# HaoruXue/spline-trajectory-optimization

Measured on AMD Instinct MI355X. Metric: min-curvature QP solves/sec (N=2000 waypoints), higher is better.
Workload: dtype f64

## Files before the change

spline_trajectory_optimization_amd/csrc/rl_device.hpp:

```cpp
#pragma once
#include <hip/hip_runtime.h>
#include "rl_sep.hpp"

namespace rl {

constexpr int kWave = 64;
constexpr int kMaxK = 5;

struct TrackDev {
  int k, n, nt, N;
  const double* t;
  const double* c0;
  const int* ell;
  const double* D;
  const int* sup;
  const double* base;
  const double* Ds;
  const double* base_s;
};

template <int K>
__device__ __forceinline__ void deboor(const double* __restrict__ t, double x, int l, int m,
                                       double (&h)[K + 1]) {
  double hh[K + 1];
// ... 195 lines not shown
      v = ring[j1];
      const double bx = v.x - px, by = v.y - py;
      const double eb = edge_side<ST>(bx, by, dx, dy);
      edge_hit<ST>(ax, ay, ea, bx, by, eb, dx, dy, j, h);
      ax = bx; ay = by; ea = eb;
      j = j1;
    }
  }
}

constexpr int kChunk = 8;
constexpr int kWinChunks = 3;
constexpr int kNear = 1;
constexpr int kWinEdges = kWinChunks * kChunk;
constexpr int kRingPad = kWinEdges + 1;
constexpr int kWinBatch = 8;

template <int BATCH = kWinBatch, bool ST = false, typename RingPtr>
__device__ __forceinline__ void scan_window(RingPtr ring, int nr, int lo, int lo_edge, double px, double py,
                                            double dx, double dy, Hit& h, const double* cmax_p,
                                            unsigned long long* counts = nullptr) {
  unsigned cand;
  {
    unsigned signs;
    double emin;
    bool sure;
    {
      const double c0 = fma(px, dy, -(py * dx));
      double2 v = ring[lo];
      const double e0 = fma(v.x, dy, fma(-v.y, dx, -c0));
      signs = (unsigned)__double2hiint(e0) >> 31;
      emin = fabs(e0);
#pragma unroll
      for (int q0 = 0; q0 < kWinEdges; q0 += BATCH) {
        double2 w[BATCH];
#pragma unroll
        for (int u = 0; u < BATCH; ++u) w[u] = ring[lo + q0 + u + 1];
#pragma unroll
        for (int u = 0; u < BATCH; ++u) {
          const double eb = fma(w[u].x, dy, fma(-w[u].y, dx, -c0));
          signs = __builtin_amdgcn_alignbit(signs, (unsigned)__double2hiint(eb), 31);
// ... 18 lines not shown
        double2 w[BATCH];
#pragma unroll
        for (int u = 0; u < BATCH; ++u) w[u] = ring[lo + q0 + u + 1];
#pragma unroll
        for (int u = 0; u < BATCH; ++u) {
          const double eb = edge_side<ST>(w[u].x - px, w[u].y - py, dx, dy);
          signs = __builtin_amdgcn_alignbit(signs, (unsigned)__double2hiint(eb), 31);
          emin = fmin(emin, fabs(eb));
        }
        if constexpr (BATCH != kWinBatch) __builtin_amdgcn_sched_barrier(0);
      }
      sure = emin != 0.0;
    }
    cand = __builtin_bitreverse32((signs ^ (signs >> 1)) & 0xFFFFFFu) >> 8;
    if (!sure) cand = 0xFFFFFFu;
    const bool sides_known = !__any(!sure);
    static_assert(kWinEdges == 24 && kWinEdges % BATCH == 0, "window scan is unrolled in whole batches; the candidate word holds 24 edges");
    while (__any(cand != 0u)) {
#ifdef RL_STAMPS
      if (counts) counts[2] += 1;
#endif
      if (cand != 0u) {
        const int q = __ffs((int)cand) - 1;
        cand &= cand - 1u;
        const int j = lo + q, je = lo_edge + q;
        const double2 va = ring[j], vb = ring[j + 1];
        const double ax = va.x - px, ay = va.y - py, bx = vb.x - px, by = vb.y - py;
        if (sides_known) edge_cross<ST>(ax, ay, bx, by, dx, dy, je >= nr ? je - nr : je, h);
        else edge_hit<ST>(ax, ay, edge_side<ST>(ax, ay, dx, dy), bx, by, edge_side<ST>(bx, by, dx, dy), dx, dy,
                          je >= nr ? je - nr : je, h);
      }
    }
  }
}

constexpr int kStage = 96;
constexpr int kStageBatch = 8;
static_assert(kStage >= kWinEdges + 1 + 64 && kStage <= 104, "a stretch holds the windows of 64 consecutive chunk starts; two DMA instructions fill it");
constexpr int kStageSlots = kStage + kStage / kChunk;
__device__ __forceinline__ int stage_slot(int v) { return v + (v >> 3); }

__device__ __forceinline__ void stage_issue(const double2* ring, int nr, int base, double2* stg, int lane) {
  static_assert(kStageSlots > kWave && kStageSlots <= 2 * kWave, "two instructions cover the stretch");
#pragma unroll
  for (int t0 = 0; t0 <= kStageSlots - kWave; t0 += kStageSlots - kWave) {
    const int t = t0 + lane;
    const int v = t - t / 9;
    int idx = base + (v < kStage ? v : kStage - 1);
    if (idx >= nr) idx -= nr;
    __builtin_amdgcn_global_load_lds((const __attribute__((address_space(1))) void*)(ring + idx),
                                     (__attribute__((address_space(3))) void*)(stg + t0), 16, 0, 0);
  }
}
struct StagedWindow {
  const double2* p;
  __device__ __forceinline__ double2 operator[](int k) const { return p[k + (k >> 3)]; }
};
__device__ __forceinline__ void stage_wait() {
  asm volatile("s_waitcnt vmcnt(0)" ::: "memory");
  __builtin_amdgcn_fence(__ATOMIC_ACQUIRE, "wavefront");
}
__device__ __forceinline__ int window_start(int hint, int nchunk) {
  int cs = hint / kChunk - 1;
  if (cs < 0) cs += nchunk;
  return cs * kChunk;
}

__device__ __forceinline__ int stage_prefetch(const double2* ring, int nr, int nchunk, bool active, int hint, double2* stg, int lane) {
  const unsigned long long m = __ballot(active && hint >= 0 && hint < nr);
  const int first = m ? __ffsll((long long)m) - 1 : 0;
  const int lo = __builtin_amdgcn_readlane(window_start(hint, nchunk), first);
  const int base = m ? lo : 0;
  asm volatile("s_waitcnt lgkmcnt(0)" ::: "memory");
  stage_issue(ring, nr, base, stg, lane);
  return base;
}

template <bool ST = false, typename RingPtr>
__device__ __forceinline__ Hit search_ring_brute(RingPtr ring, int nr, double px, double py,
                                                 double dx, double dy) {
  Hit h{INFINITY, 0.0, kNoEdge};
  scan_edges<ST>(ring, nr, 0, nr, px, py, dx, dy, h);
  return h;
}


template <bool ST = false, typename RingPtr, typename CirclePtr>
__device__ __forceinline__ Hit search_ring_culled(RingPtr ring, int nr, CirclePtr circ, int nchunk,
                                                  double px, double py, double dx, double dy,
// ... 46 lines not shown
    v = Op::f(v, __hiloint2double(hi_, lo_));                                                                   \
  }
  RL_BFLY(0x041F) RL_BFLY(0x081F) RL_BFLY(0x101F) RL_BFLY(0x201F) RL_BFLY(0x401F)
#undef RL_BFLY
  const int other = (((int)threadIdx.x ^ 32) & 63) << 2;
  const int lo_ = __builtin_amdgcn_ds_bpermute(other, __double2loint(v));
  const int hi_ = __builtin_amdgcn_ds_bpermute(other, __double2hiint(v));
  return Op::f(v, __hiloint2double(hi_, lo_));
}
__device__ __forceinline__ double wave_max_bfly(double v) { return wave_reduce_bfly<OpMax>(v); }
__device__ __forceinline__ double wave_min_bfly(double v) { return wave_reduce_bfly<OpMin>(v); }
__device__ __forceinline__ double wave_sum(double v) { return wave_reduce<OpSum>(v); }
__device__ __forceinline__ double wave_max(double v) { return wave_reduce<OpMax>(v); }
__device__ __forceinline__ double wave_min(double v) { return wave_reduce<OpMin>(v); }

template <bool STAGED = false, bool ST = false, typename RingPtr, typename CirclePtr>
__device__ __forceinline__ Hit search_ring_windowed(RingPtr ring, int nr, CirclePtr circ,
                                                    CirclePtr sep, int nchunk, bool active, int hint,
                                                    double px, double py, double dx, double dy,
                                                    double dlen, const double* cmax, bool skip_guard = false,
                                                    unsigned long long* stamps = nullptr,
                                                    double2* stg = nullptr, int staged_base = -1) {
  const int lane = threadIdx.x & (kWave - 1);
  Hit h{INFINITY, 0.0, kNoEdge};
  const bool windowed = active && hint >= 0 && hint < nr;
  const int lo = window_start(hint, nchunk);
#ifdef RL_STAMPS
  unsigned long long w0 = 0, w1 = 0;
  asm volatile("s_memtime %0\n\ts_waitcnt lgkmcnt(0)" : "=s"(w0) :: "memory");
#endif
  if constexpr (!STAGED) {
    if (windowed) scan_window<kWinBatch, ST>(ring, nr, lo, lo, px, py, dx, dy, h, cmax);
  } else {
    bool todo = windowed;
    int base = staged_base;
    if (base >= 0) stage_wait();
    for (;;) {
      if (base >= 0) {
        int off = lo - base;
        if (off < 0) off += nr;
        if (todo && (off & (kChunk - 1)) == 0 && off + kWinEdges + 1 <= kStage) {
          scan_window<kStageBatch, ST>(StagedWindow{stg + stage_slot(off)}, nr, 0, lo, px, py, dx, dy, h, cmax, stamps);
          todo = false;
        }
      }
      const unsigned long long left = __ballot(todo);
      if (left == 0ull) break;
      base = __builtin_amdgcn_readlane(lo, __ffsll((long long)left) - 1);
      asm volatile("s_waitcnt lgkmcnt(0)" ::: "memory");
      stage_issue(reinterpret_cast<const double2*>(ring), nr, base, stg, lane);
      stage_wait();
    }
  }
#ifdef RL_STAMPS
  asm volatile("s_waitcnt vmcnt(0)\n\ts_memtime %0\n\ts_waitcnt lgkmcnt(0)" : "=s"(w1) :: "memory");
  if (stamps) stamps[0] += w1 - w0;
#endif
  if (skip_guard) return h;
  const bool found = h.best <= 1.0;
  const double di = active ? ((found ? h.best * dlen : dlen) * (1.0 + 1e-9) + 1e-9) : 0.0;
  auto chunk_in_window = [&](int c) {
    const int e0 = c * kChunk;
    const int cnt = min(kChunk, nr - e0);
    int off = e0 - lo;
    if (off < 0) off += nr;
// ... 67 lines not shown
```

spline_trajectory_optimization_amd/csrc/rl_host.hpp:

```cpp
#pragma once

#include "../../include/rl_mincurv.h"

#include <hip/hip_runtime.h>

#include <mutex>
#include <string>
#include <utility>
#include <vector>

namespace {

thread_local std::string g_err;

int fail(int code, const std::string& msg) {
  g_err = msg;
  return code;
}

#define RL_HIP(expr)                                                                      \
  do {                                                                                    \
    hipError_t _e = (expr);                                                               \
    if (_e != hipSuccess) {                                                               \
      return fail(RL_ERR_HIP, std::string(#expr) + ": " + hipGetErrorString(_e));         \
// ... 23 lines not shown
};

}

struct rl_ctx {
  int device = 0;
  hipStream_t stream = nullptr;
  hipEvent_t ev0 = nullptr, ev1 = nullptr;
  int max_lds = 65536;
  int num_cu = 0;
  bool force_global_v1 = false;
  int arith = RL_ARITH_REFERENCE;
  bool arith_explicit = false;
  int np_raise_at_start = 0;
  int qss_kernel = -1, qss_df_waves = 4, qss_df_bail_at = 0, qss_df_redo = 1;
  int tables_search = RL_SEARCH_WINDOWED, tables_rings_global = 0;
  int frenet_search = 1;
  void* arena = nullptr;
  size_t arena_cap = 0;
  hipEvent_t arena_ev = nullptr;
  hipStream_t arena_stream = nullptr;
  bool arena_busy = false;
  static constexpr int kMaxGroups = 8;
  hipStream_t aux_stream[kMaxGroups - 1] = {};
  hipEvent_t ev_fork = nullptr, ev_join[kMaxGroups - 1] = {};
  hipStream_t poll_stream = nullptr;
  hipEvent_t ev_chunk[kMaxGroups] = {}, ev_poll[2] = {nullptr, nullptr};
  double* poll_host = nullptr;
  size_t poll_cap = 0;
  bool mt_hes_sweep = false;
// ... 207 lines not shown
```

spline_trajectory_optimization_amd/csrc/rl_mincurv.hip:

```cpp
#include "rl_host.hpp"

#include <algorithm>
#include <cmath>
#include <cstdio>
#include <cstdlib>
#include <cstring>
#include <type_traits>

#include "rl_kernels.hpp"
#include "rl_sweep.hpp"
#include "rl_qss_df.hpp"
#include "rl_global.hpp"
#include "rl_global2.hpp"
#include "rl_global_xy.hpp"
#include "rl_dtrack.hpp"
#include "rl_mintime.hpp"
#include "rl_bicycle.hpp"
#include "rl_region.hpp"
#include "rl_tables.hpp"
#include "rl_pose_tables.hpp"
#include "rl_spline_fit.hpp"
#include "rl_frenet.hpp"

namespace {
// ... 78 lines not shown
  int want = B >= 2 * ctx->num_cu ? 0 : 1;
  if (force && (force[0] == '0' || force[0] == '1')) want = force[0] == '1' ? 0 : 1;
  if (const char* r = getenv("RL_FORCE_RESIDENCY")) if (r[0] >= '0' && r[0] <= '2') want = r[0] - '0';
  if (strict && want == 2) want = 0;
  rl::SweepLds in = rl::sweep_lds_layout(n, N, nL, nR, Residency::Lds, joint, strict);
  if (want == 1 && in.total * sizeof(double) > (size_t)ctx->max_lds) want = 0;
  if (want == 2) {
    rl::SweepLds mid = rl::sweep_lds_layout(n, N, nL, nR, Residency::CrossingsLds, joint);
    if (mid.total * sizeof(double) > (size_t)ctx->max_lds) want = 0;
  }
  p.residency = want == 1 ? Residency::Lds : want == 2 ? Residency::CrossingsLds : Residency::Global;
  rl::SweepLds L = rl::sweep_lds_layout(n, N, nL, nR, p.residency, joint, strict);
  p.lds_bytes = L.total * sizeof(double);
  const size_t per_sample_arrays = rl::sweep_keeps_table_xy(joint, strict) ? 3 : 2;
  p.gscratch_doubles = (p.residency != Residency::Global ? 0 : per_sample_arrays * ((N + 1) & ~1) * (strict ? 2 : 1)) +
                       (p.residency == Residency::Lds ? 0 : (size_t)2 * (nL + rl::kRingPad) + (size_t)2 * (nR + rl::kRingPad));
  return p;
}

constexpr bool kRecordSteps = true;
template <int K, rl::Driver DRIVER, rl::Arith ARITH, bool DUMP = false>
int launch_sweep_in(const rl_ctx* ctx, const SweepPlan& p, const rl::SweepArgs& a) {
  using rl::Residency; using rl::SweepConfig;
  const dim3 grid(a.B), block(rl::kSweepThreads);
  return p.residency == Residency::Lds
             ? launch(ctx, rl::k_sweep<SweepConfig<K, Residency::Lds, DRIVER, ARITH, DUMP>>, grid, block, p.lds_bytes, a)
             : launch(ctx, rl::k_sweep<SweepConfig<K, Residency::Global, DRIVER, ARITH, DUMP>>, grid, block, p.lds_bytes, a);
}

int launch_sweep(const rl_ctx* ctx, int k, const SweepPlan& p, const rl::SweepArgs& a, bool joint = false, bool strict = false,
                 bool lite = false) {
// ... 208 lines not shown
    return fail(RL_ERR_ARG, "arith must be RL_ARITH_DEFAULT, RL_ARITH_FAST, RL_ARITH_REFERENCE or RL_ARITH_BRANCH");
  ctx->arith = arith;
  ctx->arith_explicit = true;
  return RL_OK;
}

int rl_ctx_get_arith(const rl_ctx* ctx) { return ctx ? (ctx->arith_explicit ? ctx->arith : RL_ARITH_DEFAULT) : RL_ERR_ARG; }

int rl_ctx_set_option(rl_ctx* ctx, const char* name, int value) {
  if (!ctx || !name) return fail(RL_ERR_ARG, "null argument");
  const std::string k(name);
  if (k == "qss_kernel") { if (value < -1 || value > 1) return fail(RL_ERR_ARG, "qss_kernel: -1 (auto), 0 (list order), 1 (dataflow)"); ctx->qss_kernel = value; }
  else if (k == "qss_df_waves") { if (value != 1 && value != 2 && value != 4) return fail(RL_ERR_ARG, "qss_df_waves: 1, 2 or 4"); ctx->qss_df_waves = value; }
  else if (k == "qss_df_bail_at") { if (value < 0) return fail(RL_ERR_ARG, "qss_df_bail_at >= 0"); ctx->qss_df_bail_at = value; }
  else if (k == "qss_df_redo") { if (value != 0 && value != 1) return fail(RL_ERR_ARG, "qss_df_redo: 0 or 1"); ctx->qss_df_redo = value; }
  else if (k == "tables_search") { if (value < RL_SEARCH_BRUTE || value > RL_SEARCH_WINDOWED) return fail(RL_ERR_ARG, "tables_search: RL_SEARCH_BRUTE, _CULLED or _WINDOWED"); ctx->tables_search = value; }
  else if (k == "tables_rings") { if (value != 0 && value != 1) return fail(RL_ERR_ARG, "tables_rings: 0 (LDS where they fit) or 1 (arena)"); ctx->tables_rings_global = value; }
  else if (k == "frenet_search") { if (value != 0 && value != 1) return fail(RL_ERR_ARG, "frenet_search: 0 (table bound for every point) or 1 (from the previous point's piece)"); ctx->frenet_search = value; }
  else return fail(RL_ERR_ARG, "unknown option '" + k + "'");
  return RL_OK;
}

int rl_ctx_set_numpy_raise(rl_ctx* ctx, int on) {
  if (!ctx) return fail(RL_ERR_ARG, "ctx is null");
  ctx->np_raise_at_start = on ? 1 : 0;
  return RL_OK;
}

int rl_debug_cr_heading(rl_ctx* ctx, const double* dx, const double* dy, int n, double* out) {
  if (!ctx || !dx || !dy || !out || n <= 0) return fail(RL_ERR_ARG, "bad argument");
// ... 221 lines not shown
    RL_HIP(hipSetDevice(ctx->device));
    if (int rc = ensure_strict_tables(ctx, trk)) return rc;
  }
  rl::SweepArgs a;
  std::memset(&a, 0, sizeof(a));
  a.tr = trk->dev();
  a.B = B;
  a.form = form;
  a.in = in_dev;
  Bounds bd;
  if (int rc = resolve_bounds(trk, form, in_dev, bd)) return rc;
  a.ringL = bd.ringL; a.ringR = bd.ringR; a.nL = bd.nL; a.nR = bd.nR;
  a.max_iter = max_iter;
  for (int j = 0; j < max_iter && !i_start_rows; ++j) a.i_start[j] = i_start[j];
  a.ctrl0 = ctrl0; a.i_start_rows = i_start_rows;
  a.search = search;
  a.max_dist = 100.0;
#ifdef RL_ABLATION
  if (const char* dbg = getenv("RL_DEBUG_FLAGS")) a.debug = atoi(dbg);
#endif
#ifdef RL_STAMPS
  const bool dbg_ok = true;
#else
  const bool dbg_ok = !strict;
#endif
  if (g_dbg_instances > 0 && (joint || k == 5) && dbg_ok && !from) {
    const int ninst = std::min(g_dbg_instances, B);
    size_t need = joint ? (size_t)max_iter * (size_t)(i_max - i_min) * (48 + 9 * rl::kJointRowsPerThread * 256 + 2 * n)
                        : (size_t)ninst * max_iter * 2 * (size_t)(i_max - i_min) * (rl::kSweepDumpHead + 2 * n);
#ifdef RL_STAMPS
    need = std::max(need, (size_t)B * 4 * 17);
#endif
    a.dbg_instances = ninst;
    if (g_dbg_len < need) {
      if (g_dbg_buf) (void)hipFree(g_dbg_buf);
      RL_HIP(hipMalloc(reinterpret_cast<void**>(&g_dbg_buf), need * sizeof(double)));
      g_dbg_len = need;
    }
    RL_HIP(hipMemsetAsync(g_dbg_buf, 0, need * sizeof(double), ctx->stream));
    a.dbg = g_dbg_buf;
  }
  a.out_ctrl = out_ctrl; a.out_xy = out_xy; a.out_points = out_points;
  a.n_success = n_success; a.status = status;
  RL_HIP(hipSetDevice(ctx->device));
  SweepPlan p = plan_sweep(ctx, n, N, a.nL, a.nR, B, joint, strict);
  if (p.lds_bytes > (size_t)ctx->max_lds) return fail(RL_ERR_UNSUPPORTED, "problem does not fit LDS");
// ... 1203 lines not shown
```

spline_trajectory_optimization_amd/csrc/rl_sweep.hpp:

```cpp
#pragma once
#include "rl_kernels.hpp"

namespace rl {

constexpr int kJointRowsPerThread = 3;

struct SweepArgs {
  TrackDev tr;
  int B;
  int form;
  const double* in;
  const double2* ringL;
  const double2* ringR;
  int nL, nR;
  int max_iter;
  int i_start[32];
  int search;
  double max_dist;
  double* out_ctrl;
  double* out_xy;
  double* out_points;
  int* n_success;
  int* status;
  double* gscratch;
  size_t gscratch_stride;
  double* dbg;
  int dbg_instances;
  int debug;
  int np_raise_at_start;
  double* aux;
  size_t aux_stride;
  int* n_raised;
  int* raise_flag;
  const double* ctrl0;
  const int* i_start_rows;
};

#ifdef RL_STAMPS
#define RL_STAMP(var) do { __builtin_amdgcn_sched_barrier(0); asm volatile("s_memtime %0\n\ts_waitcnt lgkmcnt(0)" : "=s"(var) :: "memory"); __builtin_amdgcn_sched_barrier(0); } while (0)
#define RL_STAMP_ADD(slot, t1, t0) st_acc[slot] += (t1) - (t0)
#define RL_STRICT_COUNTS st_cnt
#define RL_FSTAMP(slot) do { RL_STAMP(sf1); st_fine[slot] += sf1 - sf0; sf0 = sf1; } while (0)
#else
#define RL_STAMP(var) do { } while (0)
#define RL_STAMP_ADD(slot, t1, t0) do { } while (0)
#define RL_STRICT_COUNTS nullptr
#define RL_FSTAMP(slot) do { } while (0)
#endif

#ifdef RL_ABLATION
#define RL_ABLATE(a, bit) (((a).debug & (bit)) != 0)
#else
#define RL_ABLATE(a, bit) false
#endif

enum class Residency { Lds, Global, CrossingsLds };

struct SweepLds {
  int cpad, nLp, nRp, ncL, ncR;
  size_t off_cx, off_cy, off_red, off_sL, off_sR, off_rL, off_rR, off_cL, off_cR, off_pL, off_pR, off_hint, off_joint, off_stage,
         off_c12, off_terms, off_pxy, total;
};
__host__ __device__ constexpr bool sweep_keeps_table_xy(bool joint, bool strict) { return strict && !joint; }
constexpr int kSweepWaves = 4;
constexpr int kSweepThreads = kWave * kSweepWaves;
constexpr int kTermChunk = 256;
constexpr int kTermStride = kTermChunk + 2;
constexpr int kC12Doubles = 4 * (2 * kMaxK) + 8;
constexpr int kRedCoordMax = 194;
constexpr int kRedRadiusMax = 192;

__host__ __device__ inline SweepLds sweep_lds_layout(int n, int N, int nL, int nR, Residency residency,
                                                     bool joint = false, bool strict = false) {
  const bool rings_in_lds = residency == Residency::Lds, sigma_in_lds = residency != Residency::Global;
  SweepLds L;
  L.cpad = (n + 1) & ~1;
  L.nLp = nL; L.nRp = nR;
  L.ncL = (nL + kChunk - 1) / kChunk;
  L.ncR = (nR + kChunk - 1) / kChunk;
// ... 55 lines not shown
};
template <Residency RESIDENCY, Arith ARITH = Arith::Fast>
struct SweepConfigWindowFrom : SweepConfig<5, RESIDENCY, Driver::Window, ARITH, false> {
  static_assert(RESIDENCY != Residency::CrossingsLds, "the sliding-window driver: all-LDS or all-global residency");
  static constexpr bool from = true;
};

template <class Cfg>
__global__ __launch_bounds__(kSweepThreads, Cfg::workgroups_per_cu) void k_sweep(SweepArgs a) {
  constexpr int K = Cfg::K, BLOCK = kSweepThreads, NW = kSweepWaves;
  constexpr bool RINGS_LDS = Cfg::residency == Residency::Lds, SIGMA_LDS = Cfg::residency != Residency::Global;
  constexpr bool JOINT = Cfg::driver == Driver::Window, DUMP = Cfg::DUMP;
  constexpr bool STRICT = Cfg::arith != Arith::Fast, RAISE = Cfg::arith == Arith::ReferenceRaise, LITE = Cfg::arith == Arith::Branch;
  constexpr bool STAGED = !RINGS_LDS;
  constexpr bool FROM = Cfg::from;
  if constexpr (RAISE) { if (!a.raise_flag || a.raise_flag[blockIdx.x] == 0) return; }
#ifdef RL_STAMPS
  unsigned long long st_entry = 0;
  RL_STAMP(st_entry);
#endif
  extern __shared__ __attribute__((aligned(16))) unsigned char smem_raw[];
  double* smem = reinterpret_cast<double*>(smem_raw);
  const TrackDev& tr = a.tr;
  const int n = tr.n, N = tr.N;
  const int b = blockIdx.x;
  const int tid = threadIdx.x;
  const int lane = tid % kWave, wave = tid / kWave;
  const SweepLds L = sweep_lds_layout(n, N, a.nL, a.nR, Cfg::residency, JOINT, STRICT);
  double2* stgL = reinterpret_cast<double2*>(smem + L.off_stage) + (STAGED ? wave * 2 * kStageSlots : 0);
  double2* stgR = stgL + kStageSlots;
// ... 106 lines not shown
          m = v <= 0x1p+1000 ? fmax(m, v) : INFINITY;
          rm = o[2] <= 0x1p+1000 ? fmax(rm, o[2]) : INFINITY;
        }
        m = wave_max_bfly(m);
        rm = wave_max_bfly(rm);
        if (lane == 0) { red[kRedCoordMax] = m; red[kRedRadiusMax] = rm; }
      }
      __syncthreads();
      const double rmax = red[kRedRadiusMax];
      for (int c = tid; c < L.ncL + L.ncR; c += BLOCK) {
        const bool left = c < L.ncL;
        const int cc = left ? c : c - L.ncL;
        (left ? sepL : sepR)[cc] = chunk_separation(left ? circL : circR, left ? L.ncL : L.ncR, cc, kNear, rmax);
      }
      __syncthreads();
    }
  }

  double* jq = smem + L.off_joint;
  unsigned char* outside = reinterpret_cast<unsigned char*>(jq + 128);
  int* n_outside = reinterpret_cast<int*>(jq + 127);
  auto note_outside = [&](int i, double px, double py, double ndx, double ndy, double sl, double sr) {
    const double Lx = px + sl * ndx, Ly = py + sl * ndy;
    const double Rx = px + sr * (-ndx), Ry = py + sr * (-ndy);
    const bool out = fmin(Lx, Rx) > px || fmax(Lx, Rx) < px || fmin(Ly, Ry) > py || fmax(Ly, Ry) < py;
    const int was = outside[i];
    if ((int)out != was) { outside[i] = out ? 1 : 0; atomicAdd(n_outside, out ? 1 : -1); }
  };
  auto note_outside_pts = [&](int i, double px, double py, double2 Lp, double2 Rp) {
    const bool out = fmin(Lp.x, Rp.x) > px || fmax(Lp.x, Rp.x) < px || fmin(Lp.y, Rp.y) > py || fmax(Lp.y, Rp.y) < py;
    const int was = outside[i];
    if ((int)out != was) { outside[i] = out ? 1 : 0; atomicAdd(n_outside, out ? 1 : -1); }
  };
  if (JOINT) {
    for (int i = tid; i < N; i += BLOCK) outside[i] = 0;
    if (tid == 0) *n_outside = 0;
    __syncthreads();
  }

#ifdef RL_STAMPS
  unsigned long long st_cnt[4] = {0, 0, 0, 0};
  unsigned long long st_fine[8] = {0, 0, 0, 0, 0, 0, 0, 0}, sf0 = 0, sf1 = 0;
#endif
  unsigned char* degen = (RAISE && a.aux) ? reinterpret_cast<unsigned char*>(a.aux + (size_t)b * a.aux_stride + 2 * L.cpad) : nullptr;
  int* n_degen = reinterpret_cast<int*>(red + 190);
  bool flag_mode = false;
  bool saw_degenerate = false;
  auto refresh = [&](int i0, int i1, int j0, int j1, int mode, int l_first = -1, bool from_base = false) {
    const int m0 = i1 - i0, m1 = j1 - j0, m = m0 + m1;
    const double* cmax = red + kRedCoordMax;
    if constexpr (STRICT) {
      int delta = 0;
      auto point = [&](int i, double& px, double& py, cr::Heading& hd, bool flags, auto&& in_heading) {
#pragma clang fp contract(off)
        const int l = tr.ell[i];
        double t0[K + 1], t1[K + 1];
// ... 37 lines not shown
#endif
      };
      if (mode == 2) {
        const int nwt = (m + kWave - 1) / kWave;
        for (int wt = wave; wt < nwt; wt += NW) {
          const int r = wt * kWave + lane;
          const bool active = r < m;
          const int i = active ? (r < m0 ? i0 + r : j0 + (r - m0)) : (m0 > 0 ? i0 : j0);
          double px, py; cr::Heading hd;
#ifdef RL_STAMPS
          RL_STAMP(sf0);
#endif
          int baseL = -1, baseR = -1;
          auto prefetch = [&]() {
            if constexpr (STAGED) {
              baseL = stage_prefetch(reinterpret_cast<const double2*>(rL), nL, L.ncL, active, (int)hints[i], stgL, lane);
              baseR = stage_prefetch(reinterpret_cast<const double2*>(rR), nR, L.ncR, active, (int)hints[Npad + i], stgR, lane);
            }
          };
          if (from_base) {
            const double* bs = tr.base_s;
            px = bs[i]; py = bs[(size_t)N + i];
            hd.cl = bs[(size_t)2 * N + i]; hd.sl = bs[(size_t)3 * N + i];
            hd.cr = bs[(size_t)4 * N + i]; hd.sr = bs[(size_t)5 * N + i];
            hd.yaw = 0.0;
            prefetch();
          } else {
            point(i, px, py, hd, flag_mode && active, prefetch);
          }
          RL_FSTAMP(0);
          const double dLx = a.max_dist * hd.cl, dLy = a.max_dist * hd.sl;
          const double dRx = a.max_dist * hd.cr, dRy = a.max_dist * hd.sr;
          const Hit hl = search_ring_windowed<STAGED, true>(rL, nL, circL, sepL, L.ncL, active, (int)hints[i], px, py,
                                                            dLx, dLy, a.max_dist, cmax, false, RL_STRICT_COUNTS, stgL, baseL);
          RL_FSTAMP(1);
          const Hit hr = search_ring_windowed<STAGED, true>(rR, nR, circR, sepR, L.ncR, active, (int)hints[Npad + i], px, py,
                                                            dRx, dRy, a.max_dist, cmax, false, RL_STRICT_COUNTS, stgR, baseR);
          RL_FSTAMP(2);
          if (active) {
            const double2 Lp = make_double2(uf_madd(px, hl.best_s, dLx), uf_madd(py, hl.best_s, dLy));
            const double2 Rp = make_double2(uf_madd(px, hr.best_s, dRx), uf_madd(py, hr.best_s, dRy));
            bL[i] = Lp; bR[i] = Rp;
            if constexpr (TABLE_XY) pXY[i] = make_double2(px, py);
            hints[i] = (unsigned short)(hl.edge == kNoEdge ? 0xFFFF : hl.edge);
            hints[Npad + i] = (unsigned short)(hr.edge == kNoEdge ? 0xFFFF : hr.edge);
            if (JOINT) note_outside_pts(i, px, py, Lp, Rp);
          }
        }
        if constexpr (RAISE) { if (delta != 0) atomicAdd(n_degen, delta); }
        return;
      }
      for (int task = tid; task < 2 * m; task += BLOCK) {
// ... 26 lines not shown
      }
      return;
    }
    if (mode == 2) {
      const int nwt = (m + kWave - 1) / kWave;
      for (int wt = wave; wt < nwt; wt += NW) {
        const int r = wt * kWave + lane;
        const bool active = r < m;
        const int i = active ? (r < m0 ? i0 + r : j0 + (r - m0)) : (m0 > 0 ? i0 : j0);
        const int l = (l_first >= 0 && wt == wave && r < m0) ? l_first : tr.ell[i];
#ifdef RL_STAMPS
        RL_STAMP(sf0);
#endif
        int baseL = -1, baseR = -1;
        if constexpr (STAGED) {
          baseL = stage_prefetch(reinterpret_cast<const double2*>(rL), nL, L.ncL, active, (int)hints[i], stgL, lane);
          baseR = stage_prefetch(reinterpret_cast<const double2*>(rR), nR, L.ncR, active, (int)hints[Npad + i], stgR, lane);
        }
        CurvePoint<K, 1> c;
        eval_sample<K, 1>(tr, cx, cy, i, l, c);
        double dx, dy, inv_s2;
        scaled_normal(c.dx, c.dy, a.max_dist, dx, dy, inv_s2);
        RL_FSTAMP(0);
        const bool skip = RL_ABLATE(a, 2);
#ifdef RL_STAMPS
        unsigned long long ws[2] = {0, 0};
        const Hit hl = search_ring_windowed<STAGED>(rL, nL, circL, sepL, L.ncL, active, (int)hints[i], c.x, c.y,
                                                    dx, dy, a.max_dist, cmax, skip, ws, stgL, baseL);
        RL_FSTAMP(1);
        const Hit hr = search_ring_windowed<STAGED>(rR, nR, circR, sepR, L.ncR, active, (int)hints[Npad + i], c.x,
                                                    c.y, -dx, -dy, a.max_dist, cmax, skip, ws, stgR, baseR);
        RL_FSTAMP(2);
        st_fine[4] += ws[0];
#else
        const Hit hl = search_ring_windowed<STAGED>(rL, nL, circL, sepL, L.ncL, active, (int)hints[i], c.x, c.y,
                                                    dx, dy, a.max_dist, cmax, skip, nullptr, stgL, baseL);
        const Hit hr = search_ring_windowed<STAGED>(rR, nR, circR, sepR, L.ncR, active, (int)hints[Npad + i], c.x,
                                                    c.y, -dx, -dy, a.max_dist, cmax, skip, nullptr, stgR, baseR);
#endif
        if (active) {
          sL[i] = hl.best_s;
          sR[i] = hr.best_s;
          hints[i] = (unsigned short)(hl.edge == kNoEdge ? 0xFFFF : hl.edge);
          hints[Npad + i] = (unsigned short)(hr.edge == kNoEdge ? 0xFFFF : hr.edge);
          if (JOINT) note_outside(i, c.x, c.y, dx, dy, hl.best_s, hr.best_s);
        }
        RL_FSTAMP(3);
      }
      return;
    }
    for (int task = tid; task < 2 * m; task += BLOCK) {
      const int side = task >= m;
      const int r = side ? task - m : task;
// ... 1133 lines not shown
        }
      }
      if (tid == 0 && a.n_success) a.n_success[(size_t)b * 2 * a.max_iter + 2 * it + pass] = ok_count;
    }
  }

#ifdef RL_STAMPS
  RL_STAMP(st_t1);
  if (a.dbg && lane == 0) {
    double* o = a.dbg + ((size_t)b * NW + wave) * 16;
    for (int q = 0; q < 6; ++q) o[q] = (double)st_acc[q];
    for (int q = 0; q < 8; ++q) o[8 + q] = (double)st_fine[q];
    if constexpr (STRICT) { o[11] = (double)st_cnt[3]; o[12] = (double)st_cnt[2]; o[14] = (double)st_cnt[1]; }
    o[6] = (double)(st_t1 - st_begin);
    a.dbg[(size_t)a.B * NW * 16 + (size_t)b * NW + wave] = (double)(st_begin - st_entry);
    {
      unsigned hw, xcc;
      asm volatile("s_getreg_b32 %0, hwreg(HW_REG_HW_ID)" : "=s"(hw));
      asm volatile("s_getreg_b32 %0, hwreg(HW_REG_XCC_ID)" : "=s"(xcc));
      o[7] = (double)(((hw >> 4) & 3) | (((hw >> 8) & 15) << 4) | (((hw >> 12) & 1) << 8) | (((hw >> 13) & 7) << 9) | ((xcc & 15) << 12));
      o[15] = (double)st_begin;
    }
  }
#endif
  if constexpr (STRICT && !RINGS_LDS) __syncthreads();
  if constexpr (FROM) {
    if (bad_row) {
      n_skipped = -1;
      constexpr int per_iter = JOINT ? 1 : 2;
      if (a.n_success) for (int q = tid; q < per_iter * a.max_iter; q += BLOCK) a.n_success[(size_t)b * per_iter * a.max_iter + q] = 0;
// ... 52 lines not shown
```

Measured before the change: 104,500.

## Bracket ring-edge search with precomputed per-chunk monotone cones

Precomputes, for each ring chunk, a float cone record bounding the edge directions of its 24-edge window, and stages that record alongside the ring vertices in LDS. When the ray direction lies outside the cone, the edge-side function is monotone along the window, so only four vertices around the previous hit are tested to locate the single crossing edge instead of scanning all 24. This reduces the per-sample window scan work in the staged, strict, non-joint sweep. In exchange it adds a setup pass, extra global scratch for records, and a wave-uniform fallback to the full scan whenever the cone or tolerance checks fail.

```diff
diff --git a/spline_trajectory_optimization_amd/csrc/rl_cone.hpp b/spline_trajectory_optimization_amd/csrc/rl_cone.hpp
--- /dev/null
+++ b/spline_trajectory_optimization_amd/csrc/rl_cone.hpp
@@ -0,0 +1,58 @@
+#pragma once
+#include <cmath>
+
+#if defined(__HIPCC__)
+#include <hip/hip_runtime.h>
+#define RL_CONE_FN __host__ __device__ __forceinline__
+#else
+#define RL_CONE_FN inline
+#endif
+
+namespace rl {
+
+constexpr int kConeChunk = 8;
+constexpr int kConeEdges = 24;
+
+struct ConeRec { float ax, ay, bx, by; };
+
+template <typename RingPtr>
+RL_CONE_FN ConeRec cone_record(RingPtr ring, int nr, int cs) {
+  const ConeRec invalid{0.0f, 0.0f, 0.0f, 0.0f};
+  const int j0 = cs * kConeChunk;
+  if (nr <= 2 * kConeEdges || j0 < 0 || j0 >= nr) return invalid;
+  auto vx = [&](int k) { const int t = j0 + k; return ring[t >= nr ? t - nr : t].x; };
+  auto vy = [&](int k) { const int t = j0 + k; return ring[t >= nr ? t - nr : t].y; };
+  const double rx = vx(kConeEdges) - vx(0), ry = vy(kConeEdges) - vy(0);
+  double ax = 0.0, ay = 0.0, bx = 0.0, by = 0.0;
+  bool ok = true;
+  for (int k = 0; k < kConeEdges; ++k) {
+    const double wx = vx(k + 1) - vx(k), wy = vy(k + 1) - vy(k);
+    const double wl = fabs(wx) + fabs(wy);
+    ok = ok && wl > 0x1p-500 && wl < 0x1p+500 && rx * wx + ry * wy > 0.0;
+    if (k == 0) { ax = bx = wx; ay = by = wy; }
+    if (ax * wy - ay * wx < 0.0) { ax = wx; ay = wy; }
+    if (bx * wy - by * wx > 0.0) { bx = wx; by = wy; }
+  }
+  if (!ok) return invalid;
+  const double la = sqrt(ax * ax + ay * ay), lb = sqrt(bx * bx + by * by);
+  ax /= la; ay /= la; bx /= lb; by /= lb;
+  const double turn = 0x1p-18;
+  const ConeRec r{(float)(ax + turn * ay), (float)(ay - turn * ax), (float)(bx - turn * by), (float)(by + turn * bx)};
+  const double Ax = r.ax, Ay = r.ay, Bx = r.bx, By = r.by;
+  ok = Ax * By - Ay * Bx > 0x1p-40;
+  for (int k = 0; k < kConeEdges; ++k) {
+    const double wx = vx(k + 1) - vx(k), wy = vy(k + 1) - vy(k);
+    const double lim = 0x1p-30 * (fabs(wx) + fabs(wy));
+    ok = ok && Ax * wy - Ay * wx > lim && wx * By - wy * Bx > lim;
+  }
+  return ok ? r : invalid;
+}
+
+RL_CONE_FN bool cone_monotone(const ConeRec& r, double dx, double dy) {
+  const float fx = (float)dx, fy = (float)dy;
+  const float mg = fmaxf(0x1p-12f * (fabsf(fx) + fabsf(fy)), 0x1p-80f);
+  const float ca = fmaf(r.ax, fy, -(r.ay * fx)), cb = fmaf(r.bx, fy, -(r.by * fx));
+  return ((ca > mg) & (cb > mg)) | ((ca < -mg) & (cb < -mg));
+}
+
+}
diff --git a/spline_trajectory_optimization_amd/csrc/rl_device.hpp b/spline_trajectory_optimization_amd/csrc/rl_device.hpp
--- a/spline_trajectory_optimization_amd/csrc/rl_device.hpp
+++ b/spline_trajectory_optimization_amd/csrc/rl_device.hpp
@@ -1,6 +1,7 @@
 #pragma once
 #include <hip/hip_runtime.h>
 #include "rl_sep.hpp"
+#include "rl_cone.hpp"
 
 namespace rl {
 
@@ -233,17 +234,48 @@
 constexpr int kNear = 1;
 constexpr int kWinEdges = kWinChunks * kChunk;
 constexpr int kRingPad = kWinEdges + 1;
+static_assert(kConeChunk == kChunk && kConeEdges == kWinEdges, "rl_cone.hpp describes this window");
 constexpr int kWinBatch = 8;
 
-template <int BATCH = kWinBatch, bool ST = false, typename RingPtr>
+template <int BATCH = kWinBatch, bool ST = false, bool BRACKET = false, typename RingPtr>
 __device__ __forceinline__ void scan_window(RingPtr ring, int nr, int lo, int lo_edge, double px, double py,
                                             double dx, double dy, Hit& h, const double* cmax_p,
-                                            unsigned long long* counts = nullptr) {
-  unsigned cand;
-  {
+                                            unsigned long long* counts = nullptr,
+                                            bool bracket = false, int bq = -1) {
+  unsigned cand = 0u;
+  bool sure = true, bracketed = false;
+  if constexpr (BRACKET) {
+    if (bracket) {
+      const bool inq = bq >= 1 && bq <= kWinEdges - 2;
+      const int k0 = inq ? bq - 1 : 0;
+      double2 w[4];
+#pragma unroll
+      for (int u = 0; u < 4; ++u) w[u] = ring[lo + k0 + u];
+      const ConeRec rec = ring.record();
+      const double c0 = fma(px, dy, -(py * dx));
+      const double e0 = fma(w[0].x, dy, fma(-w[0].y, dx, -c0));
+      unsigned sg = (unsigned)__double2hiint(e0) >> 31;
+      double emin = fabs(e0);
+#pragma unroll
+      for (int u = 1; u < 4; ++u) {
+        const double e = fma(w[u].x, dy, fma(-w[u].y, dx, -c0));
+        sg = __builtin_amdgcn_alignbit(sg, (unsigned)__double2hiint(e), 31);
+        emin = fmin(emin, fabs(e));
+      }
+      const double tol = 0x1p-46 * ((cmax_p[opaque_zero()] + fabs(px)) + fabs(py)) * (fabs(dx) + fabs(dy));
+      const unsigned x = (sg ^ (sg >> 1)) & 7u;
+      const bool ok = inq & (emin > tol) & (tol > 0x1p-900) & (tol < 0x1p+900) & (x != 0u) & ((x & (x - 1u)) == 0u) &
+                      cone_monotone(rec, dx, dy);
+      bracketed = !__any(!ok);
+      if (bracketed) cand = 1u << (k0 + 2 - (int)(x >> 1));
+#ifdef RL_STAMPS
+      if (counts && bracketed) { counts[3] += 1; counts[4] += 1; }
+#endif
+    }
+  }
+  if (!bracketed) {
     unsigned signs;
     double emin;
-    bool sure;
     {
       const double c0 = fma(px, dy, -(py * dx));
       double2 v = ring[lo];
@@ -292,6 +324,8 @@
     }
     cand = __builtin_bitreverse32((signs ^ (signs >> 1)) & 0xFFFFFFu) >> 8;
     if (!sure) cand = 0xFFFFFFu;
+  }
+  {
     const bool sides_known = !__any(!sure);
     static_assert(kWinEdges == 24 && kWinEdges % BATCH == 0, "window scan is unrolled in whole batches; the candidate word holds 24 edges");
     while (__any(cand != 0u)) {
@@ -318,7 +352,8 @@
 constexpr int kStageSlots = kStage + kStage / kChunk;
 __device__ __forceinline__ int stage_slot(int v) { return v + (v >> 3); }
 
-__device__ __forceinline__ void stage_issue(const double2* ring, int nr, int base, double2* stg, int lane) {
+template <bool REC = false>
+__device__ __forceinline__ void stage_issue(const double2* ring, int nr, int base, double2* stg, int lane, int rec_off = 0) {
   static_assert(kStageSlots > kWave && kStageSlots <= 2 * kWave, "two instructions cover the stretch");
 #pragma unroll
   for (int t0 = 0; t0 <= kStageSlots - kWave; t0 += kStageSlots - kWave) {
@@ -326,6 +361,7 @@
     const int v = t - t / 9;
     int idx = base + (v < kStage ? v : kStage - 1);
     if (idx >= nr) idx -= nr;
+    if constexpr (REC) { if (t - 9 * (t / 9) == 8) idx = (rec_off + (base >> 3)) + t / 9; }
     __builtin_amdgcn_global_load_lds((const __attribute__((address_space(1))) void*)(ring + idx),
                                      (__attribute__((address_space(3))) void*)(stg + t0), 16, 0, 0);
   }
@@ -333,6 +369,11 @@
 struct StagedWindow {
   const double2* p;
   __device__ __forceinline__ double2 operator[](int k) const { return p[k + (k >> 3)]; }
+  __device__ __forceinline__ ConeRec record() const {
+    const double2 r = p[2 * kChunk + 1];
+    return ConeRec{__int_as_float(__double2loint(r.x)), __int_as_float(__double2hiint(r.x)),
+                   __int_as_float(__double2loint(r.y)), __int_as_float(__double2hiint(r.y))};
+  }
 };
 __device__ __forceinline__ void stage_wait() {
   asm volatile("s_waitcnt vmcnt(0)" ::: "memory");
@@ -344,13 +385,14 @@
   return cs * kChunk;
 }
 
-__device__ __forceinline__ int stage_prefetch(const double2* ring, int nr, int nchunk, bool active, int hint, double2* stg, int lane) {
+template <bool REC = false>
+__device__ __forceinline__ int stage_prefetch(const double2* ring, int nr, int nchunk, bool active, int hint, double2* stg, int lane, int rec_off = 0) {
   const unsigned long long m = __ballot(active && hint >= 0 && hint < nr);
   const int first = m ? __ffsll((long long)m) - 1 : 0;
   const int lo = __builtin_amdgcn_readlane(window_start(hint, nchunk), first);
   const int base = m ? lo : 0;
   asm volatile("s_waitcnt lgkmcnt(0)" ::: "memory");
-  stage_issue(ring, nr, base, stg, lane);
+  stage_issue<REC>(ring, nr, base, stg, lane, rec_off);
   return base;
 }
 
@@ -427,13 +469,15 @@
 __device__ __forceinline__ double wave_max(double v) { return wave_reduce<OpMax>(v); }
 __device__ __forceinline__ double wave_min(double v) { return wave_reduce<OpMin>(v); }
 
-template <bool STAGED = false, bool ST = false, typename RingPtr, typename CirclePtr>
+template <bool STAGED = false, bool ST = false, bool BRACKET = false, typename RingPtr, typename CirclePtr>
 __device__ __forceinline__ Hit search_ring_windowed(RingPtr ring, int nr, CirclePtr circ,
                                                     CirclePtr sep, int nchunk, bool active, int hint,
                                                     double px, double py, double dx, double dy,
                                                     double dlen, const double* cmax, bool skip_guard = false,
                                                     unsigned long long* stamps = nullptr,
-                                                    double2* stg = nullptr, int staged_base = -1) {
+                                                    double2* stg = nullptr, int staged_base = -1,
+                                                    bool bracket = false, int rec_off = 0) {
+  static_assert(!BRACKET || STAGED, "the bracket path reads the record a staged stretch carries");
   const int lane = threadIdx.x & (kWave - 1);
   Hit h{INFINITY, 0.0, kNoEdge};
   const bool windowed = active && hint >= 0 && hint < nr;
@@ -453,7 +497,10 @@
         int off = lo - base;
         if (off < 0) off += nr;
         if (todo && (off & (kChunk - 1)) == 0 && off + kWinEdges + 1 <= kStage) {
-          scan_window<kStageBatch, ST>(StagedWindow{stg + stage_slot(off)}, nr, 0, lo, px, py, dx, dy, h, cmax, stamps);
+          int bq = hint - lo;
+          if (bq < 0) bq += nr;
+          scan_window<kStageBatch, ST, BRACKET>(StagedWindow{stg + stage_slot(off)}, nr, 0, lo, px, py, dx, dy, h, cmax, stamps,
+                                                bracket, bq);
           todo = false;
         }
       }
@@ -461,7 +508,7 @@
       if (left == 0ull) break;
       base = __builtin_amdgcn_readlane(lo, __ffsll((long long)left) - 1);
       asm volatile("s_waitcnt lgkmcnt(0)" ::: "memory");
-      stage_issue(reinterpret_cast<const double2*>(ring), nr, base, stg, lane);
+      stage_issue<BRACKET>(reinterpret_cast<const double2*>(ring), nr, base, stg, lane, rec_off);
       stage_wait();
     }
   }
diff --git a/spline_trajectory_optimization_amd/csrc/rl_host.hpp b/spline_trajectory_optimization_amd/csrc/rl_host.hpp
--- a/spline_trajectory_optimization_amd/csrc/rl_host.hpp
+++ b/spline_trajectory_optimization_amd/csrc/rl_host.hpp
@@ -61,6 +61,7 @@
   bool arith_explicit = false;
   int np_raise_at_start = 0;
   int qss_kernel = -1, qss_df_waves = 4, qss_df_bail_at = 0, qss_df_redo = 1;
+  int sweep_bracket = 1;
   int tables_search = RL_SEARCH_WINDOWED, tables_rings_global = 0;
   int frenet_search = 1;
   void* arena = nullptr;
diff --git a/spline_trajectory_optimization_amd/csrc/rl_mincurv.hip b/spline_trajectory_optimization_amd/csrc/rl_mincurv.hip
--- a/spline_trajectory_optimization_amd/csrc/rl_mincurv.hip
+++ b/spline_trajectory_optimization_amd/csrc/rl_mincurv.hip
@@ -116,7 +116,8 @@
   p.lds_bytes = L.total * sizeof(double);
   const size_t per_sample_arrays = rl::sweep_keeps_table_xy(joint, strict) ? 3 : 2;
   p.gscratch_doubles = (p.residency != Residency::Global ? 0 : per_sample_arrays * ((N + 1) & ~1) * (strict ? 2 : 1)) +
-                       (p.residency == Residency::Lds ? 0 : (size_t)2 * (nL + rl::kRingPad) + (size_t)2 * (nR + rl::kRingPad));
+                       (p.residency == Residency::Lds ? 0 : (size_t)2 * (nL + rl::kRingPad) + (size_t)2 * (nR + rl::kRingPad) +
+                                                            rl::sweep_cone_doubles(L.ncL, L.ncR));
   return p;
 }
 
@@ -355,6 +356,7 @@
   else if (k == "qss_df_waves") { if (value != 1 && value != 2 && value != 4) return fail(RL_ERR_ARG, "qss_df_waves: 1, 2 or 4"); ctx->qss_df_waves = value; }
   else if (k == "qss_df_bail_at") { if (value < 0) return fail(RL_ERR_ARG, "qss_df_bail_at >= 0"); ctx->qss_df_bail_at = value; }
   else if (k == "qss_df_redo") { if (value != 0 && value != 1) return fail(RL_ERR_ARG, "qss_df_redo: 0 or 1"); ctx->qss_df_redo = value; }
+  else if (k == "sweep_bracket") { if (value != 0 && value != 1) return fail(RL_ERR_ARG, "sweep_bracket: 0 or 1"); ctx->sweep_bracket = value; }
   else if (k == "tables_search") { if (value < RL_SEARCH_BRUTE || value > RL_SEARCH_WINDOWED) return fail(RL_ERR_ARG, "tables_search: RL_SEARCH_BRUTE, _CULLED or _WINDOWED"); ctx->tables_search = value; }
   else if (k == "tables_rings") { if (value != 0 && value != 1) return fail(RL_ERR_ARG, "tables_rings: 0 (LDS where they fit) or 1 (arena)"); ctx->tables_rings_global = value; }
   else if (k == "frenet_search") { if (value != 0 && value != 1) return fail(RL_ERR_ARG, "frenet_search: 0 (table bound for every point) or 1 (from the previous point's piece)"); ctx->frenet_search = value; }
@@ -606,6 +608,7 @@
   a.max_iter = max_iter;
   for (int j = 0; j < max_iter && !i_start_rows; ++j) a.i_start[j] = i_start[j];
   a.ctrl0 = ctrl0; a.i_start_rows = i_start_rows;
+  a.bracket = ctx->sweep_bracket;
   a.search = search;
   a.max_dist = 100.0;
 #ifdef RL_ABLATION
@@ -621,7 +624,7 @@
     size_t need = joint ? (size_t)max_iter * (size_t)(i_max - i_min) * (48 + 9 * rl::kJointRowsPerThread * 256 + 2 * n)
                         : (size_t)ninst * max_iter * 2 * (size_t)(i_max - i_min) * (rl::kSweepDumpHead + 2 * n);
 #ifdef RL_STAMPS
-    need = std::max(need, (size_t)B * 4 * 17);
+    need = std::max(need, (size_t)B * 4 * 19);
 #endif
     a.dbg_instances = ninst;
     if (g_dbg_len < need) {
diff --git a/spline_trajectory_optimization_amd/csrc/rl_sweep.hpp b/spline_trajectory_optimization_amd/csrc/rl_sweep.hpp
--- a/spline_trajectory_optimization_amd/csrc/rl_sweep.hpp
+++ b/spline_trajectory_optimization_amd/csrc/rl_sweep.hpp
@@ -34,6 +34,7 @@
   int* raise_flag;
   const double* ctrl0;
   const int* i_start_rows;
+  int bracket;
 };
 
 #ifdef RL_STAMPS
@@ -63,6 +64,8 @@
 };
 __host__ __device__ constexpr bool sweep_keeps_table_xy(bool joint, bool strict) { return strict && !joint; }
 constexpr int kSweepWaves = 4;
+constexpr int kConeRecExtra = kStage / kChunk;
+__host__ __device__ constexpr size_t sweep_cone_doubles(int ncL, int ncR) { return (size_t)2 * (ncL + kConeRecExtra) + (size_t)2 * (ncR + kConeRecExtra); }
 constexpr int kSweepThreads = kWave * kSweepWaves;
 constexpr int kTermChunk = 256;
 constexpr int kTermStride = kTermChunk + 2;
@@ -148,6 +151,7 @@
   constexpr bool STRICT = Cfg::arith != Arith::Fast, RAISE = Cfg::arith == Arith::ReferenceRaise, LITE = Cfg::arith == Arith::Branch;
   constexpr bool STAGED = !RINGS_LDS;
   constexpr bool FROM = Cfg::from;
+  constexpr bool BRACKET = STAGED && !JOINT && STRICT;
   if constexpr (RAISE) { if (!a.raise_flag || a.raise_flag[blockIdx.x] == 0) return; }
 #ifdef RL_STAMPS
   unsigned long long st_entry = 0;
@@ -284,8 +288,24 @@
         (left ? sepL : sepR)[cc] = chunk_separation(left ? circL : circR, left ? L.ncL : L.ncR, cc, kNear, rmax);
       }
       __syncthreads();
+      if constexpr (BRACKET) {
+        ConeRec* recs = reinterpret_cast<ConeRec*>(rR + nR + kRingPad);
+        const int mL = L.ncL + kConeRecExtra, mR = L.ncR + kConeRecExtra;
+        for (int m = tid; m < mL + mR; m += BLOCK) {
+          const bool left = m < mL;
+          const int nc = left ? L.ncL : L.ncR;
+          int cs = (left ? m : m - mL) - 1;
+          if (cs < 0) cs += nc;
+          if (cs >= nc) cs -= nc;
+          recs[m] = cone_record(const_cast<const double2*>(left ? rL : rR), left ? nL : nR, cs);
+        }
+        __syncthreads();
+      }
     }
   }
+  const int recoL = BRACKET ? (nL + kRingPad) + (nR + kRingPad) : 0;
+  const int recoR = BRACKET ? (nR + kRingPad) + (L.ncL + kConeRecExtra) : 0;
+  const bool bracket = BRACKET && a.bracket != 0;
 
   double* jq = smem + L.off_joint;
   unsigned char* outside = reinterpret_cast<unsigned char*>(jq + 128);
@@ -309,7 +329,7 @@
   }
 
 #ifdef RL_STAMPS
-  unsigned long long st_cnt[4] = {0, 0, 0, 0};
+  unsigned long long st_cnt[5] = {0, 0, 0, 0, 0};
   unsigned long long st_fine[8] = {0, 0, 0, 0, 0, 0, 0, 0}, sf0 = 0, sf1 = 0;
 #endif
   unsigned char* degen = (RAISE && a.aux) ? reinterpret_cast<unsigned char*>(a.aux + (size_t)b * a.aux_stride + 2 * L.cpad) : nullptr;
@@ -377,8 +397,8 @@
           int baseL = -1, baseR = -1;
           auto prefetch = [&]() {
             if constexpr (STAGED) {
-              baseL = stage_prefetch(reinterpret_cast<const double2*>(rL), nL, L.ncL, active, (int)hints[i], stgL, lane);
-              baseR = stage_prefetch(reinterpret_cast<const double2*>(rR), nR, L.ncR, active, (int)hints[Npad + i], stgR, lane);
+              baseL = stage_prefetch<BRACKET>(reinterpret_cast<const double2*>(rL), nL, L.ncL, active, (int)hints[i], stgL, lane, recoL);
+              baseR = stage_prefetch<BRACKET>(reinterpret_cast<const double2*>(rR), nR, L.ncR, active, (int)hints[Npad + i], stgR, lane, recoR);
             }
           };
           if (from_base) {
@@ -394,11 +414,11 @@
           RL_FSTAMP(0);
           const double dLx = a.max_dist * hd.cl, dLy = a.max_dist * hd.sl;
           const double dRx = a.max_dist * hd.cr, dRy = a.max_dist * hd.sr;
-          const Hit hl = search_ring_windowed<STAGED, true>(rL, nL, circL, sepL, L.ncL, active, (int)hints[i], px, py,
-                                                            dLx, dLy, a.max_dist, cmax, false, RL_STRICT_COUNTS, stgL, baseL);
+          const Hit hl = search_ring_windowed<STAGED, true, BRACKET>(rL, nL, circL, sepL, L.ncL, active, (int)hints[i], px, py,
+                                                            dLx, dLy, a.max_dist, cmax, false, RL_STRICT_COUNTS, stgL, baseL, bracket, recoL);
           RL_FSTAMP(1);
-          const Hit hr = search_ring_windowed<STAGED, true>(rR, nR, circR, sepR, L.ncR, active, (int)hints[Npad + i], px, py,
-                                                            dRx, dRy, a.max_dist, cmax, false, RL_STRICT_COUNTS, stgR, baseR);
+          const Hit hr = search_ring_windowed<STAGED, true, BRACKET>(rR, nR, circR, sepR, L.ncR, active, (int)hints[Npad + i], px, py,
+                                                            dRx, dRy, a.max_dist, cmax, false, RL_STRICT_COUNTS, stgR, baseR, bracket, recoR);
           RL_FSTAMP(2);
           if (active) {
             const double2 Lp = make_double2(uf_madd(px, hl.best_s, dLx), uf_madd(py, hl.best_s, dLy));
@@ -455,8 +475,8 @@
 #endif
         int baseL = -1, baseR = -1;
         if constexpr (STAGED) {
-          baseL = stage_prefetch(reinterpret_cast<const double2*>(rL), nL, L.ncL, active, (int)hints[i], stgL, lane);
-          baseR = stage_prefetch(reinterpret_cast<const double2*>(rR), nR, L.ncR, active, (int)hints[Npad + i], stgR, lane);
+          baseL = stage_prefetch<BRACKET>(reinterpret_cast<const double2*>(rL), nL, L.ncL, active, (int)hints[i], stgL, lane, recoL);
+          baseR = stage_prefetch<BRACKET>(reinterpret_cast<const double2*>(rR), nR, L.ncR, active, (int)hints[Npad + i], stgR, lane, recoR);
         }
         CurvePoint<K, 1> c;
         eval_sample<K, 1>(tr, cx, cy, i, l, c);
@@ -465,19 +485,19 @@
         RL_FSTAMP(0);
         const bool skip = RL_ABLATE(a, 2);
 #ifdef RL_STAMPS
-        unsigned long long ws[2] = {0, 0};
-        const Hit hl = search_ring_windowed<STAGED>(rL, nL, circL, sepL, L.ncL, active, (int)hints[i], c.x, c.y,
-                                                    dx, dy, a.max_dist, cmax, skip, ws, stgL, baseL);
+        unsigned long long ws[5] = {0, 0, 0, 0, 0};
+        const Hit hl = search_ring_windowed<STAGED, false, BRACKET>(rL, nL, circL, sepL, L.ncL, active, (int)hints[i], c.x, c.y,
+                                                    dx, dy, a.max_dist, cmax, skip, ws, stgL, baseL, bracket, recoL);
         RL_FSTAMP(1);
-        const Hit hr = search_ring_windowed<STAGED>(rR, nR, circR, sepR, L.ncR, active, (int)hints[Npad + i], c.x,
-                                                    c.y, -dx, -dy, a.max_dist, cmax, skip, ws, stgR, baseR);
+        const Hit hr = search_ring_windowed<STAGED, false, BRACKET>(rR, nR, circR, sepR, L.ncR, active, (int)hints[Npad + i], c.x,
+                                                    c.y, -dx, -dy, a.max_dist, cmax, skip, ws, stgR, baseR, bracket, recoR);
         RL_FSTAMP(2);
-        st_fine[4] += ws[0];
+        st_fine[4] += ws[0]; st_cnt[3] += ws[3]; st_cnt[4] += ws[4];
 #else
-        const Hit hl = search_ring_windowed<STAGED>(rL, nL, circL, sepL, L.ncL, active, (int)hints[i], c.x, c.y,
-                                                    dx, dy, a.max_dist, cmax, skip, nullptr, stgL, baseL);
-        const Hit hr = search_ring_windowed<STAGED>(rR, nR, circR, sepR, L.ncR, active, (int)hints[Npad + i], c.x,
-                                                    c.y, -dx, -dy, a.max_dist, cmax, skip, nullptr, stgR, baseR);
+        const Hit hl = search_ring_windowed<STAGED, false, BRACKET>(rL, nL, circL, sepL, L.ncL, active, (int)hints[i], c.x, c.y,
+                                                    dx, dy, a.max_dist, cmax, skip, nullptr, stgL, baseL, bracket, recoL);
+        const Hit hr = search_ring_windowed<STAGED, false, BRACKET>(rR, nR, circR, sepR, L.ncR, active, (int)hints[Npad + i], c.x,
+                                                    c.y, -dx, -dy, a.max_dist, cmax, skip, nullptr, stgR, baseR, bracket, recoR);
 #endif
         if (active) {
           sL[i] = hl.best_s;
@@ -1641,6 +1661,8 @@
     if constexpr (STRICT) { o[11] = (double)st_cnt[3]; o[12] = (double)st_cnt[2]; o[14] = (double)st_cnt[1]; }
     o[6] = (double)(st_t1 - st_begin);
     a.dbg[(size_t)a.B * NW * 16 + (size_t)b * NW + wave] = (double)(st_begin - st_entry);
+    a.dbg[(size_t)a.B * NW * 17 + (size_t)b * NW + wave] = (double)st_cnt[3];
+    a.dbg[(size_t)a.B * NW * 18 + (size_t)b * NW + wave] = (double)st_cnt[4];
     {
       unsigned hw, xcc;
       asm volatile("s_getreg_b32 %0, hwreg(HW_REG_HW_ID)" : "=s"(hw));
```

Result: faster. 106,100, median of 6 (+1.5%).
